# mrazomej/BarBay.jl

Measured on AMD Instinct MI355X. Metric: ELBO-grad steps/sec, 50k barcodes x 8 timepoints, higher is better.
Workload: dtype f64

## Files before the change

### barbay.jl_amd/csrc/bb_engine.hip

```cpp
#include "../../include/barbay_hip.h"
#include "bb_block.h"
#include "bb_persist.h"
#include "bb_resident.h"
#include "bb_stream.h"
#include "bb_inst.h"
#include "bb_hier.h"
#include "bb_ppc.h"
#include "bb_freq.h"
#include "bb_chain.h"
#include "bb_logp.h"

#include <algorithm>
#include <cmath>
#include <cstdarg>
#include <cstdio>
#include <cstdlib>
#include <cstring>
#include <ctime>
#include <string>
#include <type_traits>
#include <vector>

static thread_local char g_err[512] = "";
static int bb_fail(int code, const char* fmt, ...) {
    va_list ap;
    va_start(ap, fmt);
    vsnprintf(g_err, sizeof g_err, fmt, ap);
    va_end(ap);
    return code;
}
extern "C" const char* bb_last_error(void) { return g_err; }

#include "bb_backend.h"

extern "C" const char* bb_version(void) { return BB_BACKEND_VERSION; }

#define BB_ENTER(h) DevGuard bb_dev_guard_((h)->o.device)

struct BBTuning {
    bool no_hist_pack, no_host_tables, no_res, no_persist, no_stream, force_stream, any_parity, force_allreduce, p2p_self;
    bool no_graph, graph_collective, no_regroup, no_reorder, nb_set, lead_set;
    int nb, res_nb, ng, lead, nthr, row_l2;
};

static BBTuning read_tuning() {
    auto set = [](const char* n) { return getenv(n) != nullptr; };
    auto num = [](const char* n, int unset) { const char* v = getenv(n); return v ? atoi(v) : unset; };
    auto on = [&](const char* n) { return num(n, 0) > 0; };
    BBTuning t{};
    t.no_hist_pack = on("BB_NO_HIST_PACK");
    t.no_host_tables = on("BB_NO_HOST_TABLES");
    t.no_res = on("BB_NO_RES");
    t.no_persist = on("BB_NO_PERSIST");
    t.no_stream = on("BB_NO_STREAM");
    t.force_stream = on("BB_TUNE_STREAM");
    t.any_parity = on("BB_TUNE_AP");
    t.force_allreduce = on("BB_FORCE_ALLREDUCE");
    t.p2p_self = on("BB_P2P_SELF");
    t.no_graph = set("BB_NO_GRAPH");
    t.graph_collective = set("BB_GRAPH_COLLECTIVE");
    t.no_regroup = set("BB_NO_REGROUP");
    t.no_reorder = set("BB_NO_REORDER");
    t.nb_set = set("BB_TUNE_NB");
    t.nb = num("BB_TUNE_NB", 0);
    t.res_nb = num("BB_TUNE_RES_NB", 0);
    t.ng = num("BB_TUNE_NG", 0);
    t.lead_set = set("BB_TUNE_LEAD");
    t.lead = num("BB_TUNE_LEAD", 65);
    if (t.lead < 10 || t.lead > 100) t.lead = 100;
    t.nthr = num("BB_TUNE_NTHR", 0) >= 64 ? num("BB_TUNE_NTHR", 0) / 64 * 64 : 0;
    t.row_l2 = num("BB_TUNE_ROW_L2", 1) == 0 ? 0 : 1;
    return t;
}

enum { IMPL_TWO_KERNEL = 0, IMPL_PERSIST = 1, IMPL_RES = 2, IMPL_STREAM = 3 };
struct LaunchPlan {
    int impl = IMPL_TWO_KERNEL;
    int P = 0;
    int NB = 0, NBL = 0, nblk = 0;
    int ng = 8, pf = 0;
    bool ms = false;
    const void* fn = nullptr;
    std::string name;
    const char* why = nullptr;
};

struct DevBuf {
    double* p = nullptr;
    size_t cap = 0;
    int grow(size_t n) {
        if (cap >= n) return 0;
        if (p) dfree(p);
        p = nullptr;
        cap = 0;
        void* q = nullptr;
        int rc = dmalloc(&q, n * 8);
        if (!rc) { p = (double*)q; cap = n; }
        return rc;
    }
};
enum {
    BUF_EPS,
    BUF_DBG,
    BUF_BANDS,
    BUF_LOGP,
    BUF_CHAIN,
    BUF_COUNT
};

struct bb_handle {
    DevModel M{};
    DevState S{};
    bb_advi_opts o{};
    std::vector<bb_block_range> blocks;
    std::vector<void*> owned;
    long long dev_bytes = 0;
    int NB = 0, nthr = 0, nblk = 0, ngeno_blk = 0;
    int tile_cap = 0;
    size_t lds_doubles = 0;
    size_t lds_doubles_p0 = 0;
    size_t lds_doubles_p = 0;
    long long b_lo = 0, b_hi = 0;
    int cus = 256;
    int g_lo = 0, g_hi = 0;
// ... 1167 lines not shown

extern "C" int bb_get_owned(bb_handle* h, int64_t* idx, int64_t* n) {
    if (!h || !idx || !n) return bb_fail(BB_ERR_INVALID, "null argument");
    std::vector<std::pair<long long, long long>> rg;
    if (h->shards.empty()) owned_ranges(h, rg);
    else for (bb_handle* sh : h->shards) owned_ranges(sh, rg);
    int64_t c = 0;
    for (auto& r : rg)
        for (long long i = r.first; i < r.second; ++i) idx[c++] = h->cidx.empty() ? i : h->cidx[(size_t)i];
    *n = c;
    return BB_OK;
}

extern "C" int bb_get_permutation(bb_handle* h, int64_t* caller_index) {
    if (!h || !caller_index) return bb_fail(BB_ERR_INVALID, "null argument");
    for (long long i = 0; i < h->M.D; ++i) caller_index[i] = h->cidx.empty() ? i : h->cidx[(size_t)i];
    return BB_OK;
}

static void p2p_release(bb_handle* h);
static void group_destroy(bb_handle* g);
extern "C" void bb_destroy(bb_handle* h) {
    if (!h) return;
    if (!h->shards.empty()) { group_destroy(h); return; }
    BB_ENTER(h);
    stream_quiesce(h->stream, h->be);
    p2p_release(h);
    hostmap_free(h->hstatus);
    for (void* p : h->owned) dfree(p);
    for (DevBuf& b : h->buf) if (b.p) dfree(b.p);
    stream_close(h->stream);
    delete h;
}

extern "C" int64_t bb_num_latents(const bb_handle* h) { return h ? h->M.D : 0; }

extern "C" int bb_get_layout(const bb_handle* h, bb_block_range* blocks, int32_t* n) {
    if (!h || !blocks || !n) return bb_fail(BB_ERR_INVALID, "null argument");
    *n = (int32_t)h->blocks.size();
    for (size_t i = 0; i < h->blocks.size(); ++i) blocks[i] = h->blocks[i];
    return BB_OK;
}

static RunArgs make_args(const bb_handle* h, long long step, int sample, int S, bool apply, bool with_elbo) {
    RunArgs A;
    memset(&A, 0, sizeof A);
    A.b_lo = h->b_lo;
    A.b_hi = h->b_hi;
    A.rank = h->o.rank;
    A.world = h->o.world_size;
    A.xepoch0 = h->epoch0;
    A.spin_limit = 1u << 23;
    A.row_l2 = h->tune.row_l2;
    A.nblk = h->nblk;
    A.nblk_alloc = h->tile_cap - 8;
    A.ng = 8;
    A.par = (int)(step & 1);
    A.sample = sample;
    A.S = S;
    A.first_sample = sample == 0;
    A.last_sample = sample == S - 1;
    A.apply = apply ? 1 : 0;
    A.with_elbo = with_elbo ? 1 : 0;
    A.count_globals = h->o.rank == 0;
    A.opt = h->o.optimizer;
    A.W = h->o.window;
    A.resum_every = h->o.resum_every;
    A.elbo_every = h->o.elbo_every;
    A.eta = h->o.eta;
    A.tau = h->o.tau;
    A.pre = h->o.pre;
    A.post = h->o.post;
    A.seed = h->o.seed;
    A.elbo_const = h->elbo_const;
    if (h->use_reduce()) { A.red = h->S.totals; A.nred = 1; }
    else { A.red = h->S.partials; A.nred = h->nblk; }
    return A;
}

static int ensure_scratch(bb_handle* h) {
    if (h->S.zsv) return BB_OK;
    const size_t D = (size_t)h->M.D, n = (D + 2 + 1) & ~(size_t)1;
    double* slab = nullptr;
    int rc = dalloc(h, &slab, 7 * n);
    if (rc) return rc;
    h->S.zsv = slab; h->S.asv = slab + n; h->S.hsv = slab + 2 * n; h->S.gacc_mu = slab + 3 * n; h->S.gacc_om = slab + 4 * n;
    h->bak_mu = slab + 5 * n; h->bak_om = slab + 6 * n;
    return h->dS ? h2d(h->dS, &h->S, sizeof(DevState), h->stream) : BB_OK;
}

static int launch_sample(bb_handle* h, const RunArgs& A) {
    if (!h->S.zsv) return bb_fail(BB_ERR_DEVICE, "internal: the two-kernel step's scratch arrays were not allocated (ensure_scratch)");
    int rc = 0;
    by_kind(h->M.kind, [&](auto kindc) {
        rc = launch(h->stream, k_sample<decltype(kindc)::value>, h->nblk, h->nthr, h->lds_doubles, desc_ptr(h->dM, &h->M), desc_ptr(h->dS, &h->S), A, h->NB);
    });
    return rc;
}
static int launch_update(bb_handle* h, const RunArgs& A) {
    if (!h->S.zsv) return bb_fail(BB_ERR_DEVICE, "internal: the two-kernel step's scratch arrays were not allocated (ensure_scratch)");
    int rc = 0;
    by_kind(h->M.kind, [&](auto kindc) {
        rc = launch(h->stream, k_update<decltype(kindc)::value>, h->nblk, h->nthr, h->lds_doubles, desc_ptr(h->dM, &h->M), desc_ptr(h->dS, &h->S), A, h->NB);
    });
    return rc;
}
// ... 814 lines not shown
```

### barbay.jl_amd/csrc/bb_persist.h

```cpp
#pragma once
#include "bb_block.h"
#include <string.h>

template <int KIND>
BB_DEV BBLds bbp_layout(const BBCtx& cx, const DevModel& M, int NB) {
    if (cx.lay) return *(const BBLds*)cx.lay;
    return bb_lds_layout(M.R, M.E, KIND, M.Ttot, M.nt1, M.K, NB, cx.nthr, 1);
}

template <int P>
struct BBPst {
    bb_d2 mu[P], om[P], am[P], ao[P];
    bb_d2 a[P], h[P];
    bb_d2 hm[P], ho[P];
    long long i0[P];
    int meta[P];
    bb_f4 lo[P];
};

#ifdef BB_EMU
#define BB_PSTATE(stv, tid) ((stv)[tid])
#else
#define BB_PSTATE(stv, tid) ((stv)[0])
#endif
// ... 405 lines not shown
            }
        }
        BB_SYNC(cx);
        BB_STAMP(cx, S, 18);
        return;
    }
    BB_PASS(cx, tid) {
        if (tid < KKP) {
            const bool act = tid < KK;
            const int k = act ? tid : KK - 1;
            double s = 0.0;
            for (int m0 = 0; m0 < members; m0 += 8) {
                double v[8];
                const int n = members - m0 < 8 ? members - m0 : 8;
                if (!bb_gran_poll8(S.grow + (long long)g * KS, (unsigned)(m0 * NG * KS + k), (unsigned)(NG * KS), n, epoch, act, S.gbar + 1, A.spin_limit, v)) *ok = 0;
#pragma unroll
                for (int i = 0; i < 8; ++i) s += v[i];
            }
            if (XG) {
                if (act) for (int r = 0; r < A.world; ++r) bb_gran_st<true>(S.xgr[r] + bbx_slot(A, par, A.rank, g) * KK + k, s, epoch);
            } else if (act) bb_gran_st(S.gxrow + ((long long)par * NG + g) * KK + k, s, epoch);
        }
    }
    BB_STAMP(cx, S, 18);
}

BB_DEV void bbp_consume_tg(BBCtx& cx, const DevModel& M, const DevState& S, const RunArgs& A, const BBLds& L, int par, unsigned epoch, int* ok) {
    double* lds = cx.lds;
    const int KK = M.K + 2 * M.nt1, NG = bbp_groups(A);
    const int KKP = (KK + 63) & ~63, NQ = (NG + 7) >> 3;
    double s0 = 0.0;
    BB_PASS(cx, tid) {
        const int q = (tid >= KKP ? 1 : 0) + (tid >= 2 * KKP ? 1 : 0) + (tid >= 3 * KKP ? 1 : 0) + (tid >= 4 * KKP ? 1 : 0), kk = tid - q * KKP;
        if (q < NQ) {
            const bool act = kk < KK;
            const int k = act ? kk : KK - 1, g0 = 8 * q;
            double v[8];
            const int n = NG - g0 < 8 ? NG - g0 : 8;
            if (!bb_gran_poll8(S.gxrow + (long long)par * NG * KK, (unsigned)(g0 * KK + k), (unsigned)KK, n, epoch, act, S.gbar + 1, A.spin_limit, v)) *ok = 0;
            double s = 0.0;
#pragma unroll
            for (int i = 0; i < 8; ++i) s += v[i];
            if (q > 0) { if (act) lds[L.red + (q - 1) * KKP + kk] = s; }
            else {
#ifdef BB_EMU
                if (act) lds[L.red + 3 * KKP + kk] = s;
#else
                s0 = s;
#endif
            }
        }
    }
    BB_STAMP(cx, S, 1);
    BB_SYNC(cx);
    BB_PASS(cx, tid) {
        if (tid < KK) {
#ifdef BB_EMU
            s0 = lds[L.red + 3 * KKP + tid];
#endif
            double s = s0;
            for (int q = 1; q < NQ; ++q) s += lds[L.red + (q - 1) * KKP + tid];
            if (tid < M.K) bb_put_total(M, L, lds, tid, s);
            else lds[L.zgl + (tid - M.K)] = s;
        }
    }
    if (!(KK <= 64 && M.Ttot <= 64)) BB_SYNC(cx);
}

BB_DEV void bbp_consume_tgx(BBCtx& cx, const DevModel& M, const DevState& S, const RunArgs& A, const BBLds& L, int par, unsigned epoch, int* ok) {
    double* lds = cx.lds;
    const int KK = M.K + 2 * M.nt1, KKP = (KK + 63) & ~63, chunks = A.world;
    int NQ = cx.nthr / KKP;
    if (NQ > chunks) NQ = chunks;
    if (NQ < 1) NQ = 1;
    const bb_gran* in = S.xgr[A.rank] + (long long)par * A.world * 8 * KK;
    BB_PASS(cx, tid) {
        int q = 0;
        for (int t = KKP; t <= tid && q < NQ; t += KKP) ++q;
        const int kk = tid - q * KKP;
        if (q < NQ) {
            const bool act = kk < KK;
            const int k = act ? kk : KK - 1;
            for (int c = q; c < chunks; c += NQ) {
                double v[8];
                if (!bb_gran_poll8<true>(in, (unsigned)(c * 8 * KK + k), (unsigned)KK, 8, epoch, act, S.gbar + 1, A.spin_limit, v)) *ok = 0;
                double s = 0.0;
#pragma unroll
                for (int i = 0; i < 8; ++i) s += v[i];
                if (act) lds[L.red + c * KKP + kk] = s;
            }
        }
    }
    BB_STAMP(cx, S, 1);
    BB_SYNC(cx);
    BB_PASS(cx, tid) {
        if (tid < KK) {
            double s = lds[L.red + tid];
            for (int c = 1; c < chunks; ++c) s += lds[L.red + c * KKP + tid];
            if (tid < M.K) bb_put_total(M, L, lds, tid, s);
            else lds[L.zgl + (tid - M.K)] = s;
        }
    }
    if (!(KK <= 64 && M.Ttot <= 64)) BB_SYNC(cx);
}

BB_DEV void bb_st_sys(double* p, double v) {
#ifdef BB_EMU
// ... 293 lines not shown
```

### barbay.jl_amd/csrc/bb_resident.h

```cpp
#pragma once
#include "bb_persist.h"

#define BR_NCV 12
#if defined(BB_EMU) || defined(BR_NO_FENCE)
#define BR_SCHED_FENCE() ((void)0)
#else
#define BR_SCHED_FENCE() __builtin_amdgcn_sched_barrier(0)
#endif
#define BR_MAXT 16

struct BRSeg { long long lo, hi; int tbeg, span, blk, kind, ldsoff, r, lpb, T; double pm, iv; const double* mean_e; const double* iv_e; long long blo; int rstride, pad; };
#define BR_SEG_DOUBLES 12

struct BRLay {
    BBLds L;
    int zl, NBT;
    int zr0[BB_MAX_REP];
    int zlw, stw;
    int st[6], SU, nst;
    int eps;
    int hbuf;
    int racc;
    int racc_r[BB_MAX_REP], rw[BB_MAX_REP];
    int rowmap;
    int iG, csum;
    int rtab;
    int ftab;
    int envt;
    int gas;
    int gix;
    int seg;
    int total;
    int lpb[BB_MAX_REP];
};

#define BR_ST(Y, i) ((Y).st[0] + (i) * (Y).stw)
static inline int br_lpb(int T) { return (T + 1) / 2; }
BB_HD int br_lpb_stream(int T) { const int l = (T + 1) / 2; return l <= 1 ? 1 : (l <= 2 ? 2 : (l <= 4 ? 4 : 8)); }

static inline long long br_tile_span(const DevModel& M, long long NB, bool globals, bool stream = false) {
    long long p = 0;
    for (int r = 0; r < M.R; ++r) p = ((p + 63) & ~63ll) + NB * (stream ? br_lpb_stream(M.T[r]) : br_lpb(M.T[r]));
    if (M.kind == 0 || M.kind == 1) p += 2 * (NB * M.E / 2 + 1);
    else if (M.kind == 2) p += 4 * (NB / 2 + 1);
    else if (M.kind == 3) p += (NB / 2 + 1) + 3ll * M.R * (NB / 2 + 1);
    else p += (NB * M.E / 2 + 1) + 3ll * M.R * (NB * M.E / 2 + 1);
    if (globals) p += 2 * (M.nt1 / 2 + 1);
    return p;
}

static inline bool br_eligible(const DevModel& M) {
    if (M.kind == 2 && !M.geno_sorted) return false;
    if (M.quirk || M.Ttot > 64) return false;
    for (int r = 0; r < M.R; ++r) if (M.T[r] < 2 || M.T[r] > BR_MAXT) return false;
    return true;
}
static inline bool br_any_parity(const DevModel& M) {
    if (M.blk_lo[BK_L] & 1) return true;
    for (int r = 0; r < M.R; ++r) if ((M.T[r] & 1) || (M.off_l[r] & 1)) return true;
    return false;
}

struct BRHdr { int rowmap, tmap, wk, zgl, Lt, invS, cc, wbar, gglob, misc, part, Dt, elbt, iG, csum, ftab, rtab, envt, seg, end; };
#ifndef BB_EMU
__host__ __device__
#endif
inline constexpr BRHdr br_header(int K, int nt1, int Ttot, int R) {
    BRHdr h{};
    const int KK = K + 2 * nt1;
    int o = 0;
    h.rowmap = o;  o += K + 1;
    h.tmap = o;    o += (K + 1) / 2 + 1;
    h.wk = o;      o += KK;
    h.zgl = o;     o += 2 * nt1;
    h.Lt = o;      o += Ttot;
    h.invS = o;    o += Ttot;
    h.cc = o;      o += Ttot + 1;
    h.wbar = o;    o += Ttot + 1;
    h.gglob = o;   o += 2 * nt1;
    h.misc = o;    o += 16 + BB_MAX_REP;
    h.part = o;    o += 32;
    h.Dt = o;      o += Ttot + 1;
    h.elbt = o;    o += Ttot;
    h.iG = o;      o += Ttot;
    h.csum = o;    o += BB_MAX_REP;
    o = (o + 1) & ~1;
    h.ftab = o;    o += 2 * Ttot;
    h.rtab = o;    o += 2 * R;
    h.envt = o;    o += (Ttot + 1) / 2 + 1;
    o = (o + 1) & ~1;
    h.seg = o;     o += BR_SEG_DOUBLES * (4 + 4 * R + 1);
    h.end = (o + 1) & ~1;
    return h;
}

static inline
#ifndef BB_EMU
__host__ __device__
#endif
BRLay br_layout(const DevModel& M, int NB, int NT, int P, int xg_rows, bool own_hbuf = false, bool stream = false) {
    BRLay Y;
    const int X = (M.kind == 1) ? M.E : (M.kind == 4 ? M.E * M.R : M.R);
    const int KK = M.K + 2 * M.nt1;
    int o = 0;
    int lmax = 1;
    for (int r = 0; r < BB_MAX_REP; ++r) { Y.lpb[r] = r < M.R ? (stream ? br_lpb_stream(M.T[r]) : br_lpb(M.T[r])) : 1; if (Y.lpb[r] > lmax) lmax = Y.lpb[r]; }
    BBLds& L = Y.L;
    L = BBLds{};
    Y.NBT = 0;
    for (int r = 0; r < BB_MAX_REP; ++r) { Y.zr0[r] = Y.NBT; if (r < M.R) Y.NBT += NB * (M.T[r] + 1); }
    Y.NBT = (Y.NBT + 1) & ~1;
    if (stream) { long long sp = 0; for (int r = 0; r < M.R; ++r) sp += (long long)NB * (M.T[r] / 2); Y.NBT = (int)(2 * sp + 2); }
    {
        const BRHdr H = br_header(M.K, M.nt1, M.Ttot, M.R);
        Y.rowmap = H.rowmap; L.tmap = H.tmap; L.wk = H.wk; L.zgl = H.zgl; L.Lt = H.Lt; L.invS = H.invS; L.cc = H.cc; L.GG = H.wbar; L.wbar = H.wbar;
        L.gglob = H.gglob; L.misc = H.misc; L.part = H.part; L.Dt = H.Dt; L.elbt = H.elbt; Y.iG = H.iG; Y.csum = H.csum; Y.ftab = H.ftab;
        Y.rtab = H.rtab; Y.envt = H.envt; Y.seg = H.seg; L.seg = H.seg;
        o = H.end;
    }
    Y.zlw = stream ? 1 : 2;
    Y.zl = o;      o += Y.zlw * Y.NBT;
    Y.SU = NB * X;
    Y.nst = stream ? (M.kind <= 1 ? 2 : 4) : (M.kind <= 1 ? 3 : 6);
    Y.stw = 2 * Y.SU;
// ... 6 lines not shown
    Y.racc = o;
    int racc_total = 0;
    for (int r = 0; r < BB_MAX_REP; ++r) {
        Y.racc_r[r] = Y.racc + racc_total;
        Y.rw[r] = r < M.R ? (stream ? (NT / (M.R == 1 ? 16 : 64)) * Y.lpb[r] : (int)(((long long)NB * Y.lpb[r] + 63) & ~63ll)) : 0;
        if (r < M.R) racc_total += BR_NCV * (Y.rw[r] + 4);
    }
    int busy;
    if (stream) {
        Y.hbuf = Y.racc;
        busy = racc_total > 2 * Y.SU ? racc_total : 2 * Y.SU;
        o += busy;
        Y.eps = o;     o += NT / 2;
    } else if (own_hbuf) {
        Y.eps = Y.racc;
        busy = 2 * P * NT;
        o += racc_total > busy ? racc_total : busy;
        o = (o + 1) & ~1;
        Y.hbuf = o;    o += 4 * P * NT;
    } else {
        Y.hbuf = Y.racc;
        Y.eps = Y.hbuf + 4 * P * NT;
        busy = 6 * P * NT;
        o += racc_total > busy ? racc_total : busy;
    }
    { const int nch = xg_rows / 8 > 5 ? xg_rows / 8 : 5;
      L.red = o;     o += 2 * 128 + nch * ((KK + 63) & ~63) + 16; }
    (void)lmax;
    L.total = Y.total = (o + 1) & ~1;
    return Y;
}

template <int P>
struct BRSt {
    bb_d2 mu[P], om[P], am[P], ao[P];
    bb_d2 a[P], h[P];
    bb_d2 z[P];
    bb_d2 lam[P];
    long long i0[P];
    int meta[P];
    int zoff[P];
    int uo[P][3];
    int pt[P];
    int rb[P];
    int thoff[P];
    unsigned cnt[P][2];
    bb_f4 lo[P];
    bb_d2 gp[P];
    bb_d2 gm[P], go[P];
    double el;
};

enum { BRM_A0 = 1 << 4, BRM_A1 = 1 << 5, BRM_VALID = 1 << 6, BRM_MUT = 1 << 7, BRM_PREV = 1 << 8, BRM_NEXT = 1 << 9 };

template <bool AP> BB_DEV bool br_pair_aligned(long long i0) { return !AP || !(i0 & 1); }
template <bool AP> BB_DEV bb_d2 br_load_pair(const double* base, long long i0, bool a0, bool a1) {
    if (a0 && a1 && br_pair_aligned<AP>(i0)) return *(const bb_d2*)(base + i0);
    return bb_d2{a0 ? base[i0] : 0.0, a1 ? base[i0 + 1] : 0.0};
}
template <bool AP> BB_DEV void br_store_pair_stream(double* base, long long i0, bool a0, bool a1, bb_d2 v) {
#ifndef BB_EMU
    if (a0 && a1 && br_pair_aligned<AP>(i0)) {
        typedef double bb_v2d __attribute__((ext_vector_type(2)));
        bb_v2d w = {v.x, v.y};
        __builtin_nontemporal_store(w, (bb_v2d*)(base + i0));
        return;
    }
    if (a0) __builtin_nontemporal_store(v.x, base + i0);
    if (a1) __builtin_nontemporal_store(v.y, base + i0 + 1);
#else
    if (a0 && a1 && br_pair_aligned<AP>(i0)) { *(bb_d2*)(base + i0) = v; return; }
    if (a0) base[i0] = v.x;
    if (a1) base[i0 + 1] = v.y;
#endif
}
template <bool AP> BB_DEV void br_store_pair(double* base, long long i0, bool a0, bool a1, bb_d2 v) {
    if (a0 && a1 && br_pair_aligned<AP>(i0)) { *(bb_d2*)(base + i0) = v; return; }
    if (a0) base[i0] = v.x;
    if (a1) base[i0 + 1] = v.y;
}

BB_HD BBTile br_tile(const DevModel& M, const RunArgs& A, int block, int NB) {
    if (A.nbl <= 0) return bb_tile(M, A, block, NB);
    const int nlead = bbp_groups(A);
    BBTile t;
    t.NB = NB;
    const int cap = block < nlead ? A.nbl : NB;
    t.b0 = block < nlead ? A.b_lo + (long long)block * A.nbl : A.b_lo + (long long)nlead * A.nbl + (long long)(block - nlead) * NB;
    long long b1 = t.b0 + cap < A.b_hi ? t.b0 + cap : A.b_hi;
    if (t.b0 > A.b_hi) t.b0 = A.b_hi;
    t.nbt = (int)(b1 > t.b0 ? b1 - t.b0 : 0);
    long long ns = M.nn - t.b0;
    t.nshift = (int)(ns < 0 ? 0 : (ns > t.nbt ? t.nbt : ns));
    t.m0 = t.b0 + t.nshift - M.nn;
    t.nmt = t.nbt - t.nshift;
    return t;
}

BB_HD BBTile br_tile_geno(const DevModel& M, const DevState& S, int block, int NB) {
    BBTile t;
    t.NB = NB;
    t.b0 = S.tile_b[block];
    t.nbt = (int)(S.tile_b[block + 1] - t.b0);
    long long ns = M.nn - t.b0;
    t.nshift = (int)(ns < 0 ? 0 : (ns > t.nbt ? t.nbt : ns));
    t.m0 = t.b0 + t.nshift - M.nn;
// ... 87 lines not shown
                    const int co = rtb[4 * s.r + 3];
                    const long long cb = (co >= 0 ? (long long)co : M.cnt_off[s.r]) + t.b0 * s.T + (long long)bl * s.T + t0;
                    st.cnt[k][0] = M.counts[cb];
                    st.cnt[k][1] = t0 + 1 < s.T ? M.counts[cb + 1] : 0u;
                }
            }
        } else {
            const int q = p - s.tbeg;
            i0 = 2 * ((s.lo >> 1) + q);
            const bool a0 = i0 >= s.lo, a1 = i0 + 1 < s.hi;
            meta |= (a0 ? BRM_A0 : 0) | (a1 ? BRM_A1 : 0) | BRM_VALID;
            st.zoff[k] = s.ldsoff + (int)(i0 - s.lo);
            st.thoff[k] = s.ldsoff;
            if (KIND == 2 && s.kind == SK_TH_R) {
                for (int x = 0; x < 2; ++x) {
                    const long long gl = (i0 - s.lo) + x;
                    int v = 0;
                    if (gl >= 0 && gl < g1 - g0) {
                        if (gl < Y.SU) v = gx[Y.SU + (int)gl];
                        else {
                            const long long g = g0 + gl;
                            const int n = M.geno_ptr[g + 1] - M.geno_ptr[g];
                            v = (n > 0 ? (int)(M.geno_mem[M.geno_ptr[g]] - t.m0) : 0) | (n << 16);
                        }
                    }
                    st.uo[k][x] = v;
                }
            } else if (s.kind < SK_GS) {
                int env = 0;
                for (int x = 0; x < 2; ++x) {
                    int j = (int)(i0 - s.lo) + x;
                    if (j < 0) j = 0;
                    const int ml = j / E, e = j - ml * E;
                    st.uo[k][x] = t.nshift + ml;
                    if (KIND == 2) env |= ((j < t.nmt ? gx[j] : 0) & 0xffff) << (16 * x);
                    else env |= e << (8 * x);
                }
                st.uo[k][2] = env;
                st.pt[k] = s.r;
            }
        }
    }
    st.i0[k] = i0;
    st.meta[k] = meta;
}

BB_HD void br_table_row(const DevModel& M, const BRLay& Y, int j, int* rm2, int* tmapj) {
    int code = 0, col = 0;
    for (int r = 0; r < M.R; ++r) {
        const int T = M.T[r], q0 = j - M.kq[r];
        if (q0 < 0 || q0 >= 6 * T - 5) continue;
        int tt, q;
        if (q0 < T) { tt = q0; q = 0; } else { tt = (q0 - T) / 5; q = 1 + (q0 - T) - 5 * tt; }
        code = Y.lpb[r] | (1 << 24);
        col = Y.racc_r[r] + ((tt & 1) * 6 + q) * (Y.rw[r] + 4) + (tt >> 1);
    }
    rm2[0] = code;
    rm2[1] = col;
    int tj = -1;
    for (int r = 0; r < M.R; ++r) { const int tt = j - M.kq[r]; if (tt >= 0 && tt < M.T[r]) tj = M.tcum[r] + tt; }
    *tmapj = tj;
}
BB_HD void br_table_time(const DevModel& M, const BBLds& L, int j, int* ft) {
    int r = 0;
    while (r + 1 < M.R && j >= M.tcum[r + 1]) ++r;
    const int tt = j - M.tcum[r], T = M.T[r];
    ft[0] = tt < T - 1 ? L.wk + M.kq[r] + T + 5 * tt : -1;
    ft[1] = M.off_t[r] + tt;
    ft[2] = tt > 0 ? 1 : 0;
    ft[3] = 0;
}
BB_HD void br_table_rep(const DevModel& M, const BRLay& Y, int r, int* rt) {
    rt[0] = M.tcum[r]; rt[1] = Y.zr0[r]; rt[2] = M.T[r];
    rt[3] = M.cnt_off[r] < (1ll << 31) ? (int)M.cnt_off[r] : -1;
}

template <int KIND>
BB_DEV void br_tile_setup(BBCtx& cx, const DevModel& M, const DevState& S, const RunArgs& A, const BRLay& Y, int NB, int ncol_or_neg) {
    double* lds = cx.lds;
    const BBLds& L = Y.L;
    const BBTile t = KIND == 2 ? br_tile_geno(M, S, cx.block, NB) : br_tile(M, A, cx.block, NB);
    const int g0 = KIND == 2 ? S.tile_g[cx.block] : 0, g1 = KIND == 2 ? S.tile_g[cx.block + 1] : 0;
    BRSeg* sg = (BRSeg*)(lds + Y.seg);
    int* li = (int*)(lds + L.misc);
    const int KK = M.K + 2 * M.nt1;
    BB_PASS(cx, tid) {
        if (S.segtab) {
            const double* src = S.segtab + (long long)cx.block * S.segtab_stride;
            const int nd = S.segtab_stride - 1;
            for (int i = tid; i < nd; i += cx.nthr) lds[Y.seg + i] = src[i];
            if (tid == 0) li[0] = ((const int*)(src + nd))[0];
        } else if (tid == 0) li[0] = br_build_segs<KIND>(sg, M, Y, t, cx.block == 0, g0, g1);
        if (tid == 0) { li[1] = bb_get_word(S.gbar + 1) == 0u ? 1 : 0; li[2] = ncol_or_neg < 0 ? t.nbt : ncol_or_neg; }
        if (tid == 0) {
            const int xcc = br_xcc_id(), NG = bbp_groups(A);
            li[4] = A.row_l2 ? 0 : -1; li[5] = xcc; li[6] = (int)A.launch_tag; li[7] = NG;
            S.xsel[cx.block] = li[4];
            if (cx.block < NG) bb_set_word64(S.xtab + cx.block, ((unsigned long long)A.launch_tag << 32) | (unsigned)xcc);
        }
        for (int k = tid; k < KK; k += cx.nthr) lds[L.wk + k] = 0.0;
        for (int i = tid; i < Y.zlw * Y.NBT; i += cx.nthr) lds[Y.zl + i] = 0.0;
        for (int i = tid; i < Y.nst * Y.stw; i += cx.nthr) lds[Y.st[0] + i] = 0.0;
        if (tid <= M.Ttot) { lds[L.cc + tid] = 0.0; lds[L.wbar + tid] = 0.0; lds[L.Dt + tid] = 0.0; }
        if (tid < M.Ttot) ((int*)(lds + Y.envt))[tid] = (KIND == 1 || KIND == 4) ? M.env_idx[tid] : 0;
        if (S.ldstab) { for (int i = tid; i < 4 * M.R; i += cx.nthr) ((int*)(lds + Y.rtab))[i] = S.ldstab[3 * M.K + 4 * M.Ttot + i]; }
        else for (int rr = tid; rr < M.R; rr += cx.nthr) br_table_rep(M, Y, rr, (int*)(lds + Y.rtab) + 4 * rr);
        if (KIND == 2) {
            int* gx = (int*)(lds + Y.gix);
            for (int j = tid; j < t.nmt; j += cx.nthr) gx[j] = M.geno_idx[t.m0 + j] - g0;
            for (int j = tid; j < g1 - g0 && j < Y.SU; j += cx.nthr) {
                const int g = g0 + j, n = M.geno_ptr[g + 1] - M.geno_ptr[g];
                gx[Y.SU + j] = (n > 0 ? (int)(M.geno_mem[M.geno_ptr[g]] - t.m0) : 0) | (n << 16);
            }
        }
    }
    BB_STAMP_RT(cx, S, 7);
    BB_SYNC(cx);
    BB_STAMP_RT(cx, S, 8);
    int* rm = (int*)(lds + Y.rowmap);
    if (S.ldstab) {
        const int K = M.K, Tt = M.Ttot, R = M.R;
        BB_PASS(cx, tid) {
            for (int i = tid; i < 2 * K; i += cx.nthr) rm[i] = S.ldstab[i];
            for (int i = tid; i < K; i += cx.nthr) ((int*)(lds + L.tmap))[i] = S.ldstab[2 * K + i];
            for (int i = tid; i < 4 * Tt; i += cx.nthr) ((int*)(lds + Y.ftab))[i] = S.ldstab[3 * K + i];
        }
    } else {
        BB_PASS(cx, tid) {
            for (int j = tid; j < M.K; j += cx.nthr) br_table_row(M, Y, j, rm + 2 * j, (int*)(lds + L.tmap) + j);
            for (int j = tid; j < M.Ttot; j += cx.nthr) br_table_time(M, L, j, (int*)(lds + Y.ftab) + 4 * j);
        }
    }
    BB_STAMP_RT(cx, S, 9);
}

template <int KIND, int P, bool AP = false>
BB_DEV void br_prologue(BBCtx& cx, const DevModel& M, const DevState& S, const RunArgs& A, const BRLay& Y, int NB, BRSt<P>* stv) {
    double* lds = cx.lds;
    const BBLds& L = Y.L;
    const BBTile t = KIND == 2 ? br_tile_geno(M, S, cx.block, NB) : br_tile(M, A, cx.block, NB);
    const int g0 = KIND == 2 ? S.tile_g[cx.block] : 0, g1 = KIND == 2 ? S.tile_g[cx.block + 1] : 0;
    const BRSeg* sg = (const BRSeg*)(lds + Y.seg);
    const int* li = (const int*)(lds + L.misc);
    br_tile_setup<KIND>(cx, M, S, A, Y, NB, -1);
    BB_PASS(cx, tid) {
        const int nseg = li[0];
        BRSt<P>& st = BB_PSTATE(stv, tid);
#pragma unroll
        for (int k = 0; k < P; ++k) {
            br_desc<KIND, P, AP>(M, Y, t, sg, nseg, g0, g1, tid + k * cx.nthr, st, k, lds);
            const long long i0 = st.i0[k];
            const int meta = st.meta[k];
            const bool a0 = meta & BRM_A0, a1 = meta & BRM_A1;
            st.mu[k] = br_load_pair<AP>(S.mu, i0, a0, a1);
            st.om[k] = br_load_pair<AP>(S.om, i0, a0, a1);
            st.am[k] = br_load_pair<AP>(S.acc_mu, i0, a0, a1);
            st.ao[k] = br_load_pair<AP>(S.acc_om, i0, a0, a1);
            st.lo[k] = bb_load_lo(S, i0, a0, a1);
            st.a[k] = st.h[k] = st.z[k] = st.lam[k] = st.gp[k] = bb_d2{0.0, 0.0};
        }
    }
    BB_STAMP_RT(cx, S, 10);
    BB_SYNC(cx);
}

template <int P> struct BRIdx { long long i0[P]; int meta[P]; };

template <int P, bool MAYODD>
#ifdef BB_EMU
static inline
#else
__device__ __attribute__((noinline))
#endif
void br_draw_call(bb_d2* eps, int nthr, int tid, unsigned long long seed, unsigned step, unsigned stream,
                  long long i0a, long long i0b, long long i0c, long long i0d, int ma, int mb, int mc, int md) {
    BRIdx<P> ix;
    { const long long i0v[4] = {i0a, i0b, i0c, i0d}; const int mv[4] = {ma, mb, mc, md};
#pragma unroll
      for (int k = 0; k < P; ++k) { ix.i0[k] = i0v[k]; ix.meta[k] = mv[k]; } }
#pragma unroll
    for (int k = 0; k < P; ++k) {
        if (!(ix.meta[k] & BRM_VALID)) continue;
        const bool odd = MAYODD && (ix.i0[k] & 1);
        double e0 = 0.0, e1 = 0.0;
#pragma nounroll
        for (int rep = 0; rep < (odd ? 2 : 1); ++rep) {
            double a, b;
            bb_normal_pair(seed, (unsigned long long)(ix.i0[k] >> 1) + (unsigned long long)rep, step, stream, &a, &b);
            if (rep == 0) { e0 = odd ? b : a; e1 = b; }
            else e1 = a;
        }
        eps[k * nthr + tid] = bb_d2{e0, e1};
    }
}

template <int KIND, int P, bool AP = false>
BB_DEV void br_draw_ahead(BBCtx& cx, const RunArgs& A, const BRLay& Y, BRSt<P>* stv, unsigned long long step, unsigned stream = 0u) {
    bb_d2* eps = (bb_d2*)(cx.lds + Y.eps);
    BB_PASS(cx, tid) {
        BRSt<P>& st = BB_PSTATE(stv, tid);
        static_assert(P <= 4, "br_draw_call takes four pair slots");
        br_draw_call<P, AP>(eps, cx.nthr, tid, A.seed, (unsigned)step, stream, st.i0[0], P > 1 ? st.i0[P > 1 ? 1 : 0] : 0, P > 2 ? st.i0[P > 2 ? 2 : 0] : 0,
                            P > 3 ? st.i0[P > 3 ? 3 : 0] : 0, st.meta[0], P > 1 ? st.meta[P > 1 ? 1 : 0] : 0, P > 2 ? st.meta[P > 2 ? 2 : 0] : 0, P > 3 ? st.meta[P > 3 ? 3 : 0] : 0);
// ... 90 lines not shown
                }
            }
        }
#pragma unroll
        for (int k = 0; k < P; ++k) {
            const int meta = st.meta[k];
            if (!(meta & BRM_VALID)) continue;
            const int kind = meta & 15;
            if (kind == SK_L) {
                double* zw = lds + Y.zl + buf * Y.NBT + st.zoff[k];
                zw[0] = st.z[k].x;
                zw[1] = st.z[k].y;
            } else if (kind < SK_GS) {
                const int raw = br_stage_raw<KIND>(kind), trn = br_stage_trn<KIND>(kind);
                double* dst = lds + BR_ST(Y, raw) + buf * Y.SU + st.zoff[k];
                if (meta & BRM_A0) dst[0] = st.z[k].x;
                if (meta & BRM_A1) dst[1] = st.z[k].y;
                if (trn >= 0) {
                    double* dw = lds + BR_ST(Y, trn) + buf * Y.SU + st.zoff[k];
                    if (meta & BRM_A0) dw[0] = st.lam[k].x;
                    if (meta & BRM_A1) dw[1] = st.lam[k].y;
                }
            } else {
                double* dst = lds + L.wk + M.K + (kind == SK_GLS ? M.nt1 : 0) + st.zoff[k];
                if (A.count_globals) {
                    if (meta & BRM_A0) dst[0] = st.z[k].x;
                    if (meta & BRM_A1) dst[1] = st.z[k].y;
                }
            }
        }
    }
    BB_STAMP_WAVE(cx, S, A, 0);
    BB_SYNC(cx);
    BB_STAMP(cx, S, 21);
}

#ifndef BB_EMU
template <int CTRL>
__device__ __forceinline__ double br_dpp(double x) {
    int lo = __double2loint(x), hi = __double2hiint(x);
    lo = __builtin_amdgcn_update_dpp(0, lo, CTRL, 0xF, 0xF, false);
    hi = __builtin_amdgcn_update_dpp(0, hi, CTRL, 0xF, 0xF, false);
    return __hiloint2double(hi, lo);
}
__device__ __forceinline__ double br_row16_sum(double s) {
    s += br_dpp<0x128>(s);
    s += br_dpp<0x124>(s);
    s += br_dpp<0x122>(s);
    s += br_dpp<0x121>(s);
    return s;
}
#endif

template <int P, bool MS = false>
BB_DEV void br_row_publish(BBCtx& cx, const DevModel& M, const DevState& S, const BRLay& Y, BRSt<P>* stv, unsigned epoch, bool want_el = false) {
    double* lds = cx.lds;
    BB_STAMP(cx, S, 23);
    const int KK = M.K + 2 * M.nt1, KS = bb_row_stride(KK);
    const int* rm = (const int*)(lds + Y.rowmap);
    const int nbt = ((const int*)(lds + Y.L.misc))[2];
    BB_PASS(cx, tid) {
        const int c = tid & 15;
        if (MS && tid == 0) {
            double e = 0.0;
            if (want_el) {
#ifdef BB_EMU
                if (stv) for (int t2 = 0; t2 < cx.nthr; ++t2) e += BB_PSTATE(stv, t2).el;
                else for (int w = 0; w < (cx.nthr + 63) / 64; ++w) e += lds[Y.L.part + w];
#else
                for (int w = 0; w < (cx.nthr >> 6); ++w) e += lds[Y.L.part + w];
#endif
            }
            lds[Y.L.wk + M.K - 2] = e;
        }
        for (int j = tid >> 4; j < M.K; j += cx.nthr >> 4) {
            if (MS && j == M.K - 2) continue;
            const int code = rm[2 * j], lpb = code & 255;
            const double* col = lds + rm[2 * j + 1];
            double s = 0.0;
#ifdef BB_EMU
            if (c == 0 && (code >> 24)) for (int e = 0; e < nbt; ++e) s += col[e * lpb];
#else
            if (code >> 24) for (int e = c; e < nbt; e += 16) s += col[e * lpb];
            s = br_row16_sum(s);
#endif
            if (c == 0) lds[Y.L.wk + j] = s;
        }
    }
    BB_SYNC(cx);
    int* li = (int*)(lds + Y.L.misc);
    BB_PASS(cx, tid) {
        if (li[4] > 0) { for (int j = tid; j < KK; j += cx.nthr) bb_gran_st_l2(S.grow + (long long)cx.block * KS + j, lds[Y.L.wk + j], epoch); }
        else for (int j = tid; j < KK; j += cx.nthr) bb_gran_st(S.grow + (long long)cx.block * KS + j, lds[Y.L.wk + j], epoch);
        if (tid == 0 && li[4] == 0) {
            int g = cx.block;
            while (g >= li[7]) g -= li[7];
            const unsigned long long v = bb_get_word64(S.xtab + g);
            if ((unsigned)(v >> 32) == (unsigned)li[6]) { li[4] = (int)(unsigned)v == li[5] ? 1 : -1; S.xsel[cx.block] = li[4]; }
        }
    }
    BB_STAMP(cx, S, 24);
    BB_STAMP_RT(cx, S, 29);
}

template <int KIND, int P, int TT> BB_DEV void br_theta_pre(BBCtx& cx, const DevModel& M, const BRLay& Y, BRSt<P>* stv, int buf);
template <int KIND, int P, bool MS = false>
BB_DEV void br_moments(BBCtx& cx, const DevModel& M, const DevState& S, const BRLay& Y, BRSt<P>* stv, int buf, unsigned epoch, bool want_el = false) {
    double* lds = cx.lds;
    if (KIND == 2) br_theta_pre<KIND, P, 0>(cx, M, Y, stv, buf);
    if (MS && want_el) {
        BB_PASS(cx, tid) {
            BRSt<P>& st = BB_PSTATE(stv, tid);
#ifdef BB_EMU
            (void)st;
#else
            double e = br_row16_sum(st.el);
            const int lo = __double2loint(e), hi = __double2hiint(e);
            double w = 0.0;
#pragma unroll
            for (int r = 0; r < 4; ++r) w += __hiloint2double(__builtin_amdgcn_readlane(hi, 16 * r), __builtin_amdgcn_readlane(lo, 16 * r));
            if ((tid & 63) == 0) lds[Y.L.part + (tid >> 6)] = w;
#endif
        }
    }
    BB_PASS(cx, tid) {
        BRSt<P>& st = BB_PSTATE(stv, tid);
#pragma unroll
        for (int k = 0; k < P; ++k) {
            const int meta = st.meta[k];
            if ((meta & 15) != SK_L) continue;
            double cv[BR_NCV];
#pragma unroll
            for (int q = 0; q < BR_NCV; ++q) cv[q] = 0.0;
            if (meta & BRM_VALID) {
            const double* zb = lds + Y.zl + buf * Y.NBT + st.zoff[k];
            const bool hn = meta & BRM_NEXT, mut = meta & BRM_MUT;
            const double z0 = st.z[k].x, z1 = st.z[k].y;
            const double zn = hn ? zb[2] : z1;
            double dm = z1 - z0, dn = zn - z1;
            cv[0] += st.lam[k].x;
            cv[6] += st.lam[k].y;
            if (mut) {
                double sm, sn, wm, wn;
                br_unit_sw<KIND>(lds, Y, buf, st.uo[k][1], KIND >= 2 ? st.thoff[k] : 0, &sm, &wm);
                if (KIND == 1 || KIND == 4) br_unit_sw<KIND>(lds, Y, buf, st.uo[k][2], KIND >= 3 ? st.thoff[k] : 0, &sn, &wn);
                else { sn = sm; wn = wm; }
                dm -= sm; dn -= sn;
                cv[1] += wm; cv[2] += wm * dm; cv[3] += wm * dm * dm;
                if (hn) { cv[7] += wn; cv[8] += wn * dn; cv[9] += wn * dn * dn; }
            } else {
                cv[4] += dm; cv[5] += dm * dm;
                if (hn) { cv[10] += dn; cv[11] += dn * dn; }
            }
            }
            {
                const BRSeg* sgk = (const BRSeg*)(lds + Y.seg) + (meta >> 12);
                const int stride = sgk->rstride;
#pragma unroll
                for (int q = 0; q < BR_NCV; ++q) lds[st.rb[k] + q * stride] = cv[q];
            }
        }
    }
    BB_SYNC(cx);
    br_row_publish<P, MS>(cx, M, S, Y, stv, epoch, want_el);
}

template <int P, bool HD>
BB_DEV void br_prefetch_slot(BBCtx& cx, const DevModel& M, const DevState& S, const RunArgs& A, const BRLay& Y, BRSt<P>* stv, int slot) {
    if (A.opt != 0) return;
    BB_PASS(cx, tid) {
        BRSt<P>& st = BB_PSTATE(stv, tid);
#pragma unroll
        for (int k = 0; k < P; ++k) {
            if (!(st.meta[k] & BRM_VALID)) continue;
#pragma unroll
            for (int which = 0; which < 2; ++which) {
                const double* src = S.hist + ((long long)slot * 2 + which) * M.Dh + (st.i0[k] - BR_HDELTA(HD, cx.lds, Y, st.meta[k]));
                bb_d2* dst = (bb_d2*)(cx.lds + Y.hbuf) + (k * 2 + which) * cx.nthr;
#ifdef BB_EMU
                dst[tid] = bb_d2{src[0], src[1]};
#else
                __builtin_amdgcn_global_load_lds((const __attribute__((address_space(1))) void*)src,
                                                 (__attribute__((address_space(3))) void*)(dst + (tid & ~63)), 16, 0, 0);
#endif
            }
        }
    }
}

template <int KIND, bool MS = false>
BB_DEV void br_finish(BBCtx& cx, const DevModel& M, const DevState& S, const BRLay& Y, const RunArgs* Ap = nullptr, bool want_el = false, int ring = 0, int smp = 0) {
    double* lds = cx.lds;
    const BBLds& L = Y.L;
    BB_STAMP(cx, S, 25);
    BB_STAMP_RT(cx, S, 30);
    BB_PASS(cx, tid) {
        for (int j = tid; j < M.Ttot; j += cx.nthr) {
            const int* ft = (const int*)(lds + Y.ftab) + 4 * j;
            const int mo = ft[0], zo = ft[1], hasprev = ft[2];
            double Dt = 0.0, c = 0.0, wb = 0.0;
            if (mo >= 0) {
                const double nn = (double)M.nn;
                const double* mm = lds + mo;
                const double M0 = mm[0], M1 = mm[1], N1 = mm[3], N2 = mm[4];
                const double sbar = lds[L.zgl + zo], ls = lds[L.zgl + M.nt1 + zo];
                wb = bb_exp(-2.0 * ls);
                c = lds[L.Lt + j + 1] - lds[L.Lt + j] - sbar;
                const double quadN = N2 - 2.0 * c * N1 + nn * c * c;
                Dt = (M1 - c * M0) + wb * (N1 - c * nn);
                lds[L.gglob + zo] = -Dt;
                lds[L.gglob + M.nt1 + zo] = wb * quadN - nn;
                if (MS && want_el) {
                    const double M2 = mm[2], quadM = M2 - 2.0 * c * M1 + c * c * M0;
                    lds[L.elbt + j] = -0.5 * (quadM + wb * quadN) - nn * ls;
                }
            } else if (MS && want_el) lds[L.elbt + j] = 0.0;
            lds[L.cc + j] = c;
// ... 438 lines not shown
```

### barbay.jl_amd/csrc/bb_types.h

```cpp
#pragma once
#include <stdint.h>

#define BB_MAX_REP 16

enum BBBlockKind {
    BK_SPOP = 0,
    BK_LSPOP = 1,
    BK_S = 2,
    BK_TT = 3,
    BK_LT = 4,
    BK_LS = 5,
    BK_L = 6,
    BK_COUNT = 7
};

#define BB_NQ 6

struct DevPrior {
    double mean, inv_var;
    const double* mean_e;
    const double* inv_var_e;
};

struct DevModel {
// ... 25 lines not shown
    const double* piv;
};

#define BB_MAX_WORLD 16

struct bb_gran;
struct DevState {
    double *mu, *om;
    double *zsv, *asv, *hsv;
    double *acc_mu, *acc_om;
    double *hist;
    const double *optc;
    float *accl;
    double *gacc_mu, *gacc_om;
    double *partials;
    double *totals;
    double *zg;
    double *ztheta;
    double *ds;
    double *gsum;
    double *geno_el;
    double *elbo_ring;
    double *elbo_sample;
    unsigned long long *ctr;
    const double *eps_in;
    unsigned *gbar;
    unsigned *hstatus;
    double *prow;
    double *xrow;
    struct bb_gran *grow, *gxrow;
    unsigned *rdy;
    int *xsel;
    unsigned long long *xtab;
    const double *segtab;
    int segtab_stride;
    const int *ldstab;
    const long long *tile_b;
    const int *tile_g;
    unsigned long long *stamps;
    double *xout[BB_MAX_WORLD];
    unsigned *xout_rdy[BB_MAX_WORLD];
    struct bb_gran *xgr[BB_MAX_WORLD];
};

#define BB_ELBO_RING 4096

struct RunArgs {
    long long b_lo, b_hi;
    int rank, world;
    unsigned xepoch0;
    unsigned spin_limit;
    unsigned launch_tag;
    int row_l2;
    int nblk;
    int nblk_alloc;
    int ng;
    int pf;
    int nbl;
    int par;
    int sample, S;
    int first_sample, last_sample;
    int apply;
    int with_elbo;
    int count_globals;
    int opt, W, resum_every, elbo_every;
    double eta, tau, pre, post;
    unsigned long long seed;
    const double* red;
    int nred;
    double elbo_const;
};
```

Measured before the change: 72020.

## Skip row-reduction work for absent neutral/mutant classes in resident tiles

Adds per-tile facts (whether the tile has neutral lineages, mutant lineages, and a once-only mutant term) and builds a compacted walk map in LDS. Row reductions and per-lineage row-buffer stores skip entries that are provably zero for the tile, and repeated mutant q=1 entries are reduced once and fanned out to their slots. It also drops one block barrier in the persistent consumer when there is a single reduction group. This adds a per-tile O(K^2) map-building pass, an extra LDS header region and an extra sync, and relies on the skipped sums really being zero or identical.

Measured after the change: 72670, median of 4. No clear change (+0.9%).

```diff
diff --git a/barbay.jl_amd/csrc/bb_engine.hip b/barbay.jl_amd/csrc/bb_engine.hip
--- a/barbay.jl_amd/csrc/bb_engine.hip
+++ b/barbay.jl_amd/csrc/bb_engine.hip
@@ -40,7 +40,7 @@
 struct BBTuning {
     bool no_hist_pack, no_host_tables, no_res, no_persist, no_stream, force_stream, any_parity, force_allreduce, p2p_self;
     bool no_graph, graph_collective, no_regroup, no_reorder, nb_set, lead_set;
-    int nb, res_nb, ng, lead, nthr, row_l2;
+    int nb, res_nb, ng, lead, nthr, row_l2, row_skip;
 };
 
 static BBTuning read_tuning() {
@@ -70,6 +70,7 @@
     if (t.lead < 10 || t.lead > 100) t.lead = 100;
     t.nthr = num("BB_TUNE_NTHR", 0) >= 64 ? num("BB_TUNE_NTHR", 0) / 64 * 64 : 0;
     t.row_l2 = num("BB_TUNE_ROW_L2", 1) == 0 ? 0 : 1;
+    { const int v = num("BB_TUNE_ROW_SKIP", 1); t.row_skip = v == 1 ? 7 : (v >> 1) & 7; }
     return t;
 }
 
@@ -1343,6 +1344,7 @@
     A.xepoch0 = h->epoch0;
     A.spin_limit = 1u << 23;
     A.row_l2 = h->tune.row_l2;
+    A.row_skip = h->tune.row_skip;
     A.nblk = h->nblk;
     A.nblk_alloc = h->tile_cap - 8;
     A.ng = 8;
diff --git a/barbay.jl_amd/csrc/bb_persist.h b/barbay.jl_amd/csrc/bb_persist.h
--- a/barbay.jl_amd/csrc/bb_persist.h
+++ b/barbay.jl_amd/csrc/bb_persist.h
@@ -481,7 +481,7 @@
         }
     }
     BB_STAMP(cx, S, 1);
-    BB_SYNC(cx);
+    if (NQ > 1 || !(A.row_skip & 4)) BB_SYNC(cx);
     BB_PASS(cx, tid) {
         if (tid < KK) {
 #ifdef BB_EMU
diff --git a/barbay.jl_amd/csrc/bb_resident.h b/barbay.jl_amd/csrc/bb_resident.h
--- a/barbay.jl_amd/csrc/bb_resident.h
+++ b/barbay.jl_amd/csrc/bb_resident.h
@@ -70,6 +70,7 @@
     const int KK = K + 2 * nt1;
     int o = 0;
     h.rowmap = o;  o += K + 1;
+    o += K + 1;
     h.tmap = o;    o += (K + 1) / 2 + 1;
     h.wk = o;      o += KK;
     h.zgl = o;     o += 2 * nt1;
@@ -182,6 +183,7 @@
 };
 
 enum { BRM_A0 = 1 << 4, BRM_A1 = 1 << 5, BRM_VALID = 1 << 6, BRM_MUT = 1 << 7, BRM_PREV = 1 << 8, BRM_NEXT = 1 << 9 };
+enum { BRF_NEUTRAL = 1, BRF_MUTANT = 2, BRF_M0_ONCE = 4 };
 
 template <bool AP> BB_DEV bool br_pair_aligned(long long i0) { return !AP || !(i0 & 1); }
 template <bool AP> BB_DEV bb_d2 br_load_pair(const double* base, long long i0, bool a0, bool a1) {
@@ -375,7 +377,7 @@
         if (q0 < 0 || q0 >= 6 * T - 5) continue;
         int tt, q;
         if (q0 < T) { tt = q0; q = 0; } else { tt = (q0 - T) / 5; q = 1 + (q0 - T) - 5 * tt; }
-        code = Y.lpb[r] | (1 << 24);
+        code = Y.lpb[r] | (q << 8) | (tt << 12) | (1 << 24);
         col = Y.racc_r[r] + ((tt & 1) * 6 + q) * (Y.rw[r] + 4) + (tt >> 1);
     }
     rm2[0] = code;
@@ -457,6 +459,49 @@
     BB_STAMP_RT(cx, S, 9);
 }
 
+template <int P> BB_DEV constexpr bool br_row_skips() { return P == 1; }
+enum { BRB_SKIP_N = 1 << 28, BRB_SKIP_M = 1 << 29, BRB_SKIP_M0 = 1 << 30, BRB_OFFSET = (1 << 28) - 1 };
+BB_DEV int* br_walkmap(double* lds, const BRLay& Y, const DevModel& M) { return (int*)(lds + Y.rowmap + (M.K + 1)); }
+template <int KIND>
+BB_DEV int br_tile_factbits(const RunArgs& A, const BBTile& t) {
+    return ((A.row_skip & 1) ? (t.nshift > 0 ? BRF_NEUTRAL : 0) | (t.nmt > 0 ? BRF_MUTANT : 0) : (BRF_NEUTRAL | BRF_MUTANT))
+           | (((A.row_skip & 2) && (KIND == 0 || KIND == 2 || KIND == 3)) ? BRF_M0_ONCE : 0);
+}
+BB_HD bool br_entry_live(int code, int facts) {
+    if (!(code >> 24)) return false;
+    const int q = (code >> 8) & 7, tt = (code >> 12) & 15;
+    if (q == 0) return true;
+    if (q <= 3) return (facts & BRF_MUTANT) && !(q == 1 && tt > 0 && (facts & BRF_M0_ONCE));
+    return (facts & BRF_NEUTRAL) != 0;
+}
+BB_DEV void br_tile_facts(BBCtx& cx, const DevModel& M, const BRLay& Y, int facts) {
+    double* lds = cx.lds;
+    const int* rm = (const int*)(lds + Y.rowmap);
+    int* wm = br_walkmap(lds, Y, M);
+    const int K = M.K;
+    BB_PASS(cx, tid) {
+        for (int j = tid; j < K; j += cx.nthr) {
+            int before = 0, all = 0;
+            for (int i = 0; i < K; ++i) { const int l = br_entry_live(rm[2 * i], facts) ? 1 : 0; all += l; before += i < j ? l : 0; }
+            const int code = rm[2 * j];
+            const bool live = br_entry_live(code, facts);
+            const int i = live ? before : all + (j - before);
+            int cnt = 1;
+            if ((code >> 24) && ((code >> 8) & 7) == 1 && (facts & BRF_MUTANT) && (facts & BRF_M0_ONCE)) {
+                cnt = 0;
+                if (((code >> 12) & 15) == 0)
+                    for (int x = 0; j + 5 * x < K; ++x) {
+                        const int cx_ = rm[2 * (j + 5 * x)];
+                        if (!(cx_ >> 24) || ((cx_ >> 8) & 7) != 1 || ((cx_ >> 12) & 15) != x) break;
+                        ++cnt;
+                    }
+            }
+            wm[2 * i] = (code & 255) | (j << 8) | (live ? 1 << 24 : 0) | (cnt << 25);
+            wm[2 * i + 1] = rm[2 * j + 1];
+        }
+    }
+}
+
 template <int KIND, int P, bool AP = false>
 BB_DEV void br_prologue(BBCtx& cx, const DevModel& M, const DevState& S, const RunArgs& A, const BRLay& Y, int NB, BRSt<P>* stv) {
     double* lds = cx.lds;
@@ -466,12 +511,19 @@
     const BRSeg* sg = (const BRSeg*)(lds + Y.seg);
     const int* li = (const int*)(lds + L.misc);
     br_tile_setup<KIND>(cx, M, S, A, Y, NB, -1);
+    const int facts = br_row_skips<P>() ? br_tile_factbits<KIND>(A, t) : (BRF_NEUTRAL | BRF_MUTANT);
+    const int rbits = ((facts & BRF_NEUTRAL) ? 0 : BRB_SKIP_N) | ((facts & BRF_MUTANT) ? 0 : BRB_SKIP_M) | ((facts & BRF_M0_ONCE) ? BRB_SKIP_M0 : 0);
+    if (br_row_skips<P>()) {
+        BB_SYNC(cx);
+        br_tile_facts(cx, M, Y, facts);
+    }
     BB_PASS(cx, tid) {
         const int nseg = li[0];
         BRSt<P>& st = BB_PSTATE(stv, tid);
 #pragma unroll
         for (int k = 0; k < P; ++k) {
             br_desc<KIND, P, AP>(M, Y, t, sg, nseg, g0, g1, tid + k * cx.nthr, st, k, lds);
+            if (br_row_skips<P>()) st.rb[k] |= rbits;
             const long long i0 = st.i0[k];
             const int meta = st.meta[k];
             const bool a0 = meta & BRM_A0, a1 = meta & BRM_A1;
@@ -668,12 +720,12 @@
 }
 #endif
 
-template <int P, bool MS = false>
+template <int P, bool MS = false, bool LIST = false>
 BB_DEV void br_row_publish(BBCtx& cx, const DevModel& M, const DevState& S, const BRLay& Y, BRSt<P>* stv, unsigned epoch, bool want_el = false) {
     double* lds = cx.lds;
     BB_STAMP(cx, S, 23);
     const int KK = M.K + 2 * M.nt1, KS = bb_row_stride(KK);
-    const int* rm = (const int*)(lds + Y.rowmap);
+    const int* rm = LIST ? br_walkmap(lds, Y, M) : (const int*)(lds + Y.rowmap);
     const int nbt = ((const int*)(lds + Y.L.misc))[2];
     BB_PASS(cx, tid) {
         const int c = tid & 15;
@@ -689,18 +741,20 @@
             }
             lds[Y.L.wk + M.K - 2] = e;
         }
-        for (int j = tid >> 4; j < M.K; j += cx.nthr >> 4) {
+        for (int i = tid >> 4; i < M.K; i += cx.nthr >> 4) {
+            const int code = rm[2 * i], lpb = code & 255, j = LIST ? (code >> 8) & 0xffff : i, used = LIST ? (code >> 24) & 1 : code >> 24;
+            const int fill = LIST ? (code >> 25) & 31 : 1;
             if (MS && j == M.K - 2) continue;
-            const int code = rm[2 * j], lpb = code & 255;
-            const double* col = lds + rm[2 * j + 1];
+            const double* col = lds + rm[2 * i + 1];
             double s = 0.0;
 #ifdef BB_EMU
-            if (c == 0 && (code >> 24)) for (int e = 0; e < nbt; ++e) s += col[e * lpb];
+            if (c == 0 && used) for (int e = 0; e < nbt; ++e) s += col[e * lpb];
+            if (c == 0) for (int x = 0; x < fill; ++x) lds[Y.L.wk + j + 5 * x] = s;
 #else
-            if (code >> 24) for (int e = c; e < nbt; e += 16) s += col[e * lpb];
+            if (used) for (int e = c; e < nbt; e += 16) s += col[e * lpb];
             s = br_row16_sum(s);
-#endif
-            if (c == 0) lds[Y.L.wk + j] = s;
+            if (c < fill) lds[Y.L.wk + j + 5 * c] = s;
+#endif
         }
     }
     BB_SYNC(cx);
@@ -772,13 +826,20 @@
             {
                 const BRSeg* sgk = (const BRSeg*)(lds + Y.seg) + (meta >> 12);
                 const int stride = sgk->rstride;
-#pragma unroll
-                for (int q = 0; q < BR_NCV; ++q) lds[st.rb[k] + q * stride] = cv[q];
+                const int skip = br_row_skips<P>() ? st.rb[k] & ~BRB_OFFSET : 0;
+                double* rb = lds + (br_row_skips<P>() ? st.rb[k] & BRB_OFFSET : st.rb[k]);
+                rb[0] = cv[0]; rb[6 * stride] = cv[6];
+                if (!(skip & BRB_SKIP_M)) {
+                    rb[stride] = cv[1]; rb[2 * stride] = cv[2]; rb[3 * stride] = cv[3];
+                    if (!(skip & BRB_SKIP_M0)) rb[7 * stride] = cv[7];
+                    rb[8 * stride] = cv[8]; rb[9 * stride] = cv[9];
+                }
+                if (!(skip & BRB_SKIP_N)) { rb[4 * stride] = cv[4]; rb[5 * stride] = cv[5]; rb[10 * stride] = cv[10]; rb[11 * stride] = cv[11]; }
             }
         }
     }
     BB_SYNC(cx);
-    br_row_publish<P, MS>(cx, M, S, Y, stv, epoch, want_el);
+    br_row_publish<P, MS, br_row_skips<P>()>(cx, M, S, Y, stv, epoch, want_el);
 }
 
 template <int P, bool HD>
diff --git a/barbay.jl_amd/csrc/bb_types.h b/barbay.jl_amd/csrc/bb_types.h
--- a/barbay.jl_amd/csrc/bb_types.h
+++ b/barbay.jl_amd/csrc/bb_types.h
@@ -101,6 +101,7 @@
     unsigned spin_limit;
     unsigned launch_tag;
     int row_l2;
+    int row_skip;
     int nblk;
     int nblk_alloc;
     int ng;
```
